# 3dlg-hcvc/tricolo

Hardware: AMD Instinct MI355X
Metric: trimodal training samples/sec (32^3 voxel + 6-view) (higher is better)
Workload: dtype f16 (f16 activation storage + f16 MFMA operands, fp32 accumulate; bf16x3 heads/GRU; within 1e-3 of the fp32 reference)

## Files before the change

tricolo_amd/csrc/conv_pw.hip:

```cpp
#include "common.h"
#include "../../include/tricolo_hip.h"
#include "conv_vox.h"

struct PwArgs {
    const void* in;
    const void* w;
    void* out;
    float* stats;
    int M, K, N, Kpad;
    int GH, GW;
    int transposed;
};

template <int N>
static __device__ __forceinline__ float pw_row_ror(float v) {
    return __builtin_bit_cast(float, __builtin_amdgcn_update_dpp(0, __builtin_bit_cast(int, v), 0x120 + N, 0xf, 0xf, false));
}

template <typename AT, int BN>
__global__ __launch_bounds__(256) void conv_pw_kernel(const PwArgs p) {
    typedef Mma<typename OpOf<AT>::E> MM;
    typedef typename MM::v8 v8;
    constexpr int TN = BN / 16, TM = 2;
    extern __shared__ __attribute__((aligned(16))) char smem[];
    const int t = threadIdx.x, lane = t & 63, wave = t >> 6, fr = lane & 15, fq = lane >> 4;
    const int NT = p.N / BN;
    const int mtile = blockIdx.x / NT, ntile = blockIdx.x - mtile * NT;
    const int K = p.K, kchunks = K >> 3;

    {
        const AT* w = (const AT*)p.w + (size_t)ntile * BN * p.Kpad;
        for (int e = t; e < BN * kchunks; e += 256) {
            const int n = e / kchunks, c = e - n * kchunks;
            const uint4 v = *(const uint4*)(w + (size_t)n * p.Kpad + c * 8);
            *(uint4*)(smem + ((size_t)n * kchunks + (c ^ (n & 7))) * 16) = v;
        }
    }
    const AT* src[TM];
    bool ok[TM];
    size_t opix[TM];
#pragma unroll
    for (int a = 0; a < TM; ++a) {
        const int m = mtile * 128 + wave * 32 + a * 16 + fr;
        ok[a] = m < p.M;
        const int mm = ok[a] ? m : 0;
        const int x = mm % p.GW, q = mm / p.GW, y = q % p.GH, n = q / p.GH;
        const size_t big = (((size_t)n * 2 * p.GH + 2 * y) * 2 * p.GW + 2 * x);
        if (!p.transposed) { src[a] = (const AT*)p.in + big * K; opix[a] = (size_t)mm * p.N; }
        else { src[a] = (const AT*)p.in + (size_t)mm * K; opix[a] = big * p.N; }
    }
    __syncthreads();

    f32x4 acc[TM][TN];
#pragma unroll
    for (int a = 0; a < TM; ++a)
#pragma unroll
        for (int b = 0; b < TN; ++b) acc[a][b] = (f32x4){0.f, 0.f, 0.f, 0.f};
    for (int k0 = 0; k0 < K; k0 += 128) {
        uint4 af[4][TM];
#pragma unroll
        for (int s = 0; s < 4; ++s)
#pragma unroll
            for (int a = 0; a < TM; ++a) {
                af[s][a] = make_uint4(0u, 0u, 0u, 0u);
                if (ok[a] && k0 + s * 32 < K) af[s][a] = *(const uint4*)(src[a] + k0 + s * 32 + fq * 8);
            }
#pragma unroll
        for (int s = 0; s < 4; ++s) {
            if (k0 + s * 32 >= K) break;
            const int c = ((k0 + s * 32) >> 3) + fq;
#pragma unroll
            for (int b = 0; b < TN; ++b) {
                const uint4 bf = *(const uint4*)(smem + ((size_t)(b * 16 + fr) * kchunks + (c ^ (fr & 7))) * 16);
#pragma unroll
                for (int a = 0; a < TM; ++a) acc[a][b] = MM::mma(__builtin_bit_cast(v8, bf), __builtin_bit_cast(v8, af[s][a]), acc[a][b]);
            }
        }
    }

    AT* const out = (AT*)p.out + ntile * BN;
    if (p.transposed) {
        const size_t dx = p.N, dy = (size_t)2 * p.GW * p.N;
        const float4 z = make_float4(0.f, 0.f, 0.f, 0.f);
#pragma unroll
        for (int a = 0; a < TM; ++a) {
            if (!ok[a]) continue;
#pragma unroll
            for (int b = 0; b < TN; ++b) {
                AT* o = out + opix[a] + b * 16 + fq * 4;
                const f32x4 v = acc[a][b];
                Act<AT>::st4(o, make_float4(v[0], v[1], v[2], v[3]));
                Act<AT>::st4(o + dx, z);
                Act<AT>::st4(o + dy, z);
                Act<AT>::st4(o + dy + dx, z);
            }
        }
        return;
    }
    f32x4 cs[TN], cq[TN];
#pragma unroll
    for (int b = 0; b < TN; ++b) { cs[b] = (f32x4){0.f, 0.f, 0.f, 0.f}; cq[b] = cs[b]; }
#pragma unroll
    for (int a = 0; a < TM; ++a) {
        if (!ok[a]) continue;
#pragma unroll
        for (int b = 0; b < TN; ++b) {
            f32x4 v = acc[a][b];
            Act<AT>::st4(out + opix[a] + b * 16 + fq * 4, make_float4(v[0], v[1], v[2], v[3]));
            v[0] = Act<AT>::rnd(v[0]); v[1] = Act<AT>::rnd(v[1]); v[2] = Act<AT>::rnd(v[2]); v[3] = Act<AT>::rnd(v[3]);
            cs[b] += v;
            cq[b] += v * v;
        }
    }
    if (!p.stats) return;
    __syncthreads();
    float* const red = (float*)smem;
#pragma unroll
    for (int b = 0; b < TN; ++b)
#pragma unroll
        for (int r = 0; r < 4; ++r) {
            float s_ = cs[b][r], q_ = cq[b][r];
            s_ += pw_row_ror<8>(s_); q_ += pw_row_ror<8>(q_);
            s_ += pw_row_ror<4>(s_); q_ += pw_row_ror<4>(q_);
            s_ += pw_row_ror<2>(s_); q_ += pw_row_ror<2>(q_);
            s_ += pw_row_ror<1>(s_); q_ += pw_row_ror<1>(q_);
            if (fr == 0) {
                const int col = b * 16 + fq * 4 + r;
                red[(wave * BN + col) * 2 + 0] = s_;
                red[(wave * BN + col) * 2 + 1] = q_;
            }
        }
    __syncthreads();
    if (t < BN) {
        float s_ = 0.f, q_ = 0.f;
#pragma unroll
        for (int w2 = 0; w2 < 4; ++w2) { s_ += red[(w2 * BN + t) * 2]; q_ += red[(w2 * BN + t) * 2 + 1]; }
        p.stats[((size_t)mtile * 2 + 0) * p.N + ntile * BN + t] = s_;
        p.stats[((size_t)mtile * 2 + 1) * p.N + ntile * BN + t] = q_;
    }
}

bool tri_internal_pw_geometry(const TriConvDesc& d, TriPwGeom* g) {
    if (tri_env_is("TRICOLO_NO_PW_CONV", '1') || d.KD != 1 || d.KH != 1 || d.KW != 1 || d.stride != 2 || d.pad_d || d.pad_h || d.pad_w || d.ID != 1 || d.OD != 1) return false;
    if (d.Cin % 64 || d.Cin > 512 || d.Cout % 64) return false;
    int transposed;
    if (d.IH == 2 * d.OH && d.IW == 2 * d.OW) transposed = 0;
    else if (d.OH == 2 * d.IH && d.OW == 2 * d.IW) transposed = 1;
    else return false;
    const int GH = transposed ? d.IH : d.OH, GW = transposed ? d.IW : d.OW;
    const long M = (long)d.B * GH * GW;
    if (M * 4 * (d.Cin > d.Cout ? d.Cin : d.Cout) * 2 >= ((long)1 << 31)) return false;
    const int mtiles = (int)((M + 127) / 128);
    const int bn = (d.Cout % 128 == 0 && (long)128 * d.Cin * 2 <= 65536 && (long)mtiles * (d.Cout / 128) >= 256) ? 128 : 64;
    g->bn = bn; g->mtiles = mtiles; g->GH = GH; g->GW = GW; g->transposed = transposed;
    return true;
}

template <typename AT>
static int pw_launch_t(const TriPwGeom& g, const PwArgs& a, hipStream_t stream) {
    const size_t smem = (size_t)g.bn * a.K * 2 > (size_t)4 * g.bn * 2 * 4 ? (size_t)g.bn * a.K * 2 : (size_t)4 * g.bn * 2 * 4;
    const int grid = g.mtiles * (a.N / g.bn);
    if (g.bn == 128) {
        static bool set = false;
        if (!set) { hipFuncSetAttribute((const void*)conv_pw_kernel<AT, 128>, hipFuncAttributeMaxDynamicSharedMemorySize, 65536); set = true; }
        conv_pw_kernel<AT, 128><<<grid, 256, smem, stream>>>(a);
    } else {
        static bool set = false;
        if (!set) { hipFuncSetAttribute((const void*)conv_pw_kernel<AT, 64>, hipFuncAttributeMaxDynamicSharedMemorySize, 65536); set = true; }
        conv_pw_kernel<AT, 64><<<grid, 256, smem, stream>>>(a);
    }
    return tri_check_launch("tri_conv(pw)");
}

int tri_internal_pw_launch(const TriPwGeom& g, int B, const void* in, const void* w, int K, int N, int Kpad, void* out, float* stats, int transposed,
                           int act_fmt, hipStream_t stream) {
    PwArgs a{};
    a.in = in; a.w = w; a.out = out; a.stats = transposed ? nullptr : stats;
    a.M = B * g.GH * g.GW; a.K = K; a.N = N; a.Kpad = Kpad; a.GH = g.GH; a.GW = g.GW; a.transposed = transposed;
    return act_fmt == TRI_FMT_F16 ? pw_launch_t<f16_t>(g, a, stream) : pw_launch_t<bf16_t>(g, a, stream);
}
```

Before: 13370.

## Prefetch A fragments, coalesce weight staging and transposed stores, add BN=32 tiles

The pointwise stride-2 conv kernel gains a DG variant for the transposed (upsampling) path. It issues the first A-fragment loads before weight staging and double-buffers the next K-chunk's loads during the MFMA loop. Weight staging is rearranged into batched 8-chunk loads, and output is staged through per-wave LDS so each lane writes full 16-byte rows plus the zero fill, giving coalesced scatter. A BN=32 tile is also picked when the grid would otherwise be small, to raise parallelism, at the cost of more register pressure and extra LDS traffic.

```diff
diff --git a/tricolo_amd/csrc/conv_pw.hip b/tricolo_amd/csrc/conv_pw.hip
--- a/tricolo_amd/csrc/conv_pw.hip
+++ b/tricolo_amd/csrc/conv_pw.hip
@@ -17,7 +17,12 @@
     return __builtin_bit_cast(float, __builtin_amdgcn_update_dpp(0, __builtin_bit_cast(int, v), 0x120 + N, 0xf, 0xf, false));
 }
 
-template <typename AT, int BN>
+template <int BN> struct PwStage {
+    static constexpr int PITCH = BN * 2 + 16;
+    static constexpr int WAVE = 32 * PITCH + 32 * 4;
+};
+
+template <typename AT, int BN, bool DG>
 __global__ __launch_bounds__(256) void conv_pw_kernel(const PwArgs p) {
     typedef Mma<typename OpOf<AT>::E> MM;
     typedef typename MM::v8 v8;
@@ -28,17 +33,9 @@
     const int mtile = blockIdx.x / NT, ntile = blockIdx.x - mtile * NT;
     const int K = p.K, kchunks = K >> 3;
 
-    {
-        const AT* w = (const AT*)p.w + (size_t)ntile * BN * p.Kpad;
-        for (int e = t; e < BN * kchunks; e += 256) {
-            const int n = e / kchunks, c = e - n * kchunks;
-            const uint4 v = *(const uint4*)(w + (size_t)n * p.Kpad + c * 8);
-            *(uint4*)(smem + ((size_t)n * kchunks + (c ^ (n & 7))) * 16) = v;
-        }
-    }
     const AT* src[TM];
     bool ok[TM];
-    size_t opix[TM];
+    unsigned opix[TM];
 #pragma unroll
     for (int a = 0; a < TM; ++a) {
         const int m = mtile * 128 + wave * 32 + a * 16 + fr;
@@ -46,8 +43,41 @@
         const int mm = ok[a] ? m : 0;
         const int x = mm % p.GW, q = mm / p.GW, y = q % p.GH, n = q / p.GH;
         const size_t big = (((size_t)n * 2 * p.GH + 2 * y) * 2 * p.GW + 2 * x);
-        if (!p.transposed) { src[a] = (const AT*)p.in + big * K; opix[a] = (size_t)mm * p.N; }
-        else { src[a] = (const AT*)p.in + (size_t)mm * K; opix[a] = big * p.N; }
+        if (!p.transposed) { src[a] = (const AT*)p.in + big * K; opix[a] = (unsigned)((size_t)mm * p.N); }
+        else { src[a] = (const AT*)p.in + (size_t)mm * K; opix[a] = (unsigned)(big * p.N); }
+    }
+#define PW_LOAD_TRIP(af, k0_)                                                                                              \
+    _Pragma("unroll") for (int s = 0; s < 4; ++s)                                                                          \
+        _Pragma("unroll") for (int a = 0; a < TM; ++a) {                                                                   \
+            af[s][a] = make_uint4(0u, 0u, 0u, 0u);                                                                         \
+            if (ok[a] && (k0_) + s * 32 < K) af[s][a] = *(const uint4*)(src[a] + (k0_) + s * 32 + fq * 8);                 \
+        }
+    uint4 cur[4][TM], nxt[4][TM];
+    if (DG) { PW_LOAD_TRIP(cur, 0) }
+    {
+        const AT* w = (const AT*)p.w + (size_t)ntile * BN * p.Kpad;
+        if (!DG) {
+            for (int e = t; e < BN * kchunks; e += 256) {
+                const int n = e / kchunks, c = e - n * kchunks;
+                const uint4 v = *(const uint4*)(w + (size_t)n * p.Kpad + c * 8);
+                *(uint4*)(smem + ((size_t)n * kchunks + (c ^ (n & 7))) * 16) = v;
+            }
+        } else {
+            const int cc = t & 7, ng = kchunks >> 3;
+#pragma unroll
+            for (int i = 0; i < BN / 32; ++i) {
+                const int n = i * 32 + (t >> 3);
+                uint4 v[8];
+#pragma unroll
+                for (int g8 = 0; g8 < 8; ++g8) {
+                    v[g8] = make_uint4(0u, 0u, 0u, 0u);
+                    if (g8 < ng) v[g8] = *(const uint4*)(w + (size_t)n * p.Kpad + (g8 * 8 + cc) * 8);
+                }
+#pragma unroll
+                for (int g8 = 0; g8 < 8; ++g8)
+                    if (g8 < ng) *(uint4*)(smem + ((size_t)n * kchunks + g8 * 8 + (cc ^ (n & 7))) * 16) = v[g8];
+            }
+        }
     }
     __syncthreads();
 
@@ -57,14 +87,9 @@
 #pragma unroll
         for (int b = 0; b < TN; ++b) acc[a][b] = (f32x4){0.f, 0.f, 0.f, 0.f};
     for (int k0 = 0; k0 < K; k0 += 128) {
-        uint4 af[4][TM];
-#pragma unroll
-        for (int s = 0; s < 4; ++s)
-#pragma unroll
-            for (int a = 0; a < TM; ++a) {
-                af[s][a] = make_uint4(0u, 0u, 0u, 0u);
-                if (ok[a] && k0 + s * 32 < K) af[s][a] = *(const uint4*)(src[a] + k0 + s * 32 + fq * 8);
-            }
+        const bool more = DG && k0 + 128 < K;
+        if (!DG) { PW_LOAD_TRIP(cur, k0) }
+        if (more) { PW_LOAD_TRIP(nxt, k0 + 128) }
 #pragma unroll
         for (int s = 0; s < 4; ++s) {
             if (k0 + s * 32 >= K) break;
@@ -73,72 +98,121 @@
             for (int b = 0; b < TN; ++b) {
                 const uint4 bf = *(const uint4*)(smem + ((size_t)(b * 16 + fr) * kchunks + (c ^ (fr & 7))) * 16);
 #pragma unroll
-                for (int a = 0; a < TM; ++a) acc[a][b] = MM::mma(__builtin_bit_cast(v8, bf), __builtin_bit_cast(v8, af[s][a]), acc[a][b]);
-            }
-        }
-    }
-
-    AT* const out = (AT*)p.out + ntile * BN;
-    if (p.transposed) {
-        const size_t dx = p.N, dy = (size_t)2 * p.GW * p.N;
-        const float4 z = make_float4(0.f, 0.f, 0.f, 0.f);
+                for (int a = 0; a < TM; ++a) acc[a][b] = MM::mma(__builtin_bit_cast(v8, bf), __builtin_bit_cast(v8, cur[s][a]), acc[a][b]);
+            }
+        }
+        if (more) {
+#pragma unroll
+            for (int s = 0; s < 4; ++s)
+#pragma unroll
+                for (int a = 0; a < TM; ++a) cur[s][a] = nxt[s][a];
+        }
+    }
+
+    if (!DG) {
+        AT* const out = (AT*)p.out + ntile * BN;
+        if (p.transposed) {
+            const size_t dx = p.N, dy = (size_t)2 * p.GW * p.N;
+            const float4 z = make_float4(0.f, 0.f, 0.f, 0.f);
+#pragma unroll
+            for (int a = 0; a < TM; ++a) {
+                if (!ok[a]) continue;
+#pragma unroll
+                for (int b = 0; b < TN; ++b) {
+                    AT* o = out + opix[a] + b * 16 + fq * 4;
+                    const f32x4 v = acc[a][b];
+                    Act<AT>::st4(o, make_float4(v[0], v[1], v[2], v[3]));
+                    Act<AT>::st4(o + dx, z);
+                    Act<AT>::st4(o + dy, z);
+                    Act<AT>::st4(o + dy + dx, z);
+                }
+            }
+            return;
+        }
+        f32x4 cs[TN], cq[TN];
+#pragma unroll
+        for (int b = 0; b < TN; ++b) { cs[b] = (f32x4){0.f, 0.f, 0.f, 0.f}; cq[b] = cs[b]; }
 #pragma unroll
         for (int a = 0; a < TM; ++a) {
             if (!ok[a]) continue;
 #pragma unroll
             for (int b = 0; b < TN; ++b) {
-                AT* o = out + opix[a] + b * 16 + fq * 4;
-                const f32x4 v = acc[a][b];
-                Act<AT>::st4(o, make_float4(v[0], v[1], v[2], v[3]));
-                Act<AT>::st4(o + dx, z);
-                Act<AT>::st4(o + dy, z);
-                Act<AT>::st4(o + dy + dx, z);
-            }
+                f32x4 v = acc[a][b];
+                Act<AT>::st4(out + opix[a] + b * 16 + fq * 4, make_float4(v[0], v[1], v[2], v[3]));
+                v[0] = Act<AT>::rnd(v[0]); v[1] = Act<AT>::rnd(v[1]); v[2] = Act<AT>::rnd(v[2]); v[3] = Act<AT>::rnd(v[3]);
+                cs[b] += v;
+                cq[b] += v * v;
+            }
+        }
+        if (!p.stats) return;
+        __syncthreads();
+        float* const red = (float*)smem;
+#pragma unroll
+        for (int b = 0; b < TN; ++b)
+#pragma unroll
+            for (int r = 0; r < 4; ++r) {
+                float s_ = cs[b][r], q_ = cq[b][r];
+                s_ += pw_row_ror<8>(s_); q_ += pw_row_ror<8>(q_);
+                s_ += pw_row_ror<4>(s_); q_ += pw_row_ror<4>(q_);
+                s_ += pw_row_ror<2>(s_); q_ += pw_row_ror<2>(q_);
+                s_ += pw_row_ror<1>(s_); q_ += pw_row_ror<1>(q_);
+                if (fr == 0) {
+                    const int col = b * 16 + fq * 4 + r;
+                    red[(wave * BN + col) * 2 + 0] = s_;
+                    red[(wave * BN + col) * 2 + 1] = q_;
+                }
+            }
+        __syncthreads();
+        if (t < BN) {
+            float s_ = 0.f, q_ = 0.f;
+#pragma unroll
+            for (int w2 = 0; w2 < 4; ++w2) { s_ += red[(w2 * BN + t) * 2]; q_ += red[(w2 * BN + t) * 2 + 1]; }
+            p.stats[((size_t)mtile * 2 + 0) * p.N + ntile * BN + t] = s_;
+            p.stats[((size_t)mtile * 2 + 1) * p.N + ntile * BN + t] = q_;
         }
         return;
     }
-    f32x4 cs[TN], cq[TN];
-#pragma unroll
-    for (int b = 0; b < TN; ++b) { cs[b] = (f32x4){0.f, 0.f, 0.f, 0.f}; cq[b] = cs[b]; }
+    __syncthreads();
+    typedef PwStage<BN> ST;
+    char* const stage = smem + wave * ST::WAVE;
+    unsigned* const spix = (unsigned*)(stage + 32 * ST::PITCH);
 #pragma unroll
     for (int a = 0; a < TM; ++a) {
-        if (!ok[a]) continue;
+        if (fq == 0) spix[a * 16 + fr] = ok[a] ? opix[a] : 0xffffffffu;
 #pragma unroll
         for (int b = 0; b < TN; ++b) {
-            f32x4 v = acc[a][b];
-            Act<AT>::st4(out + opix[a] + b * 16 + fq * 4, make_float4(v[0], v[1], v[2], v[3]));
-            v[0] = Act<AT>::rnd(v[0]); v[1] = Act<AT>::rnd(v[1]); v[2] = Act<AT>::rnd(v[2]); v[3] = Act<AT>::rnd(v[3]);
-            cs[b] += v;
-            cq[b] += v * v;
-        }
-    }
-    if (!p.stats) return;
-    __syncthreads();
-    float* const red = (float*)smem;
-#pragma unroll
-    for (int b = 0; b < TN; ++b)
-#pragma unroll
-        for (int r = 0; r < 4; ++r) {
-            float s_ = cs[b][r], q_ = cq[b][r];
-            s_ += pw_row_ror<8>(s_); q_ += pw_row_ror<8>(q_);
-            s_ += pw_row_ror<4>(s_); q_ += pw_row_ror<4>(q_);
-            s_ += pw_row_ror<2>(s_); q_ += pw_row_ror<2>(q_);
-            s_ += pw_row_ror<1>(s_); q_ += pw_row_ror<1>(q_);
-            if (fr == 0) {
-                const int col = b * 16 + fq * 4 + r;
-                red[(wave * BN + col) * 2 + 0] = s_;
-                red[(wave * BN + col) * 2 + 1] = q_;
-            }
-        }
-    __syncthreads();
-    if (t < BN) {
-        float s_ = 0.f, q_ = 0.f;
-#pragma unroll
-        for (int w2 = 0; w2 < 4; ++w2) { s_ += red[(w2 * BN + t) * 2]; q_ += red[(w2 * BN + t) * 2 + 1]; }
-        p.stats[((size_t)mtile * 2 + 0) * p.N + ntile * BN + t] = s_;
-        p.stats[((size_t)mtile * 2 + 1) * p.N + ntile * BN + t] = q_;
-    }
-}
+            const f32x4 v = acc[a][b];
+            Act<AT>::st4((AT*)(stage + (a * 16 + fr) * ST::PITCH) + b * 16 + fq * 4, make_float4(v[0], v[1], v[2], v[3]));
+        }
+    }
+    __builtin_amdgcn_fence(__ATOMIC_ACQ_REL, "workgroup");
+    __builtin_amdgcn_wave_barrier();
+    {
+        constexpr int LPR = BN / 8, RPI = 64 / LPR, NIT = 32 / RPI;
+        AT* const out = (AT*)p.out + ntile * BN + (lane % LPR) * 8;
+        const size_t dx = p.N, dy = (size_t)2 * p.GW * p.N;
+        const uint4 z = make_uint4(0u, 0u, 0u, 0u);
+        unsigned px[NIT];
+        uint4 v[NIT];
+#pragma unroll
+        for (int it = 0; it < NIT; ++it) {
+            const int r = it * RPI + lane / LPR;
+            px[it] = spix[r];
+            v[it] = *(const uint4*)(stage + r * ST::PITCH + (lane % LPR) * 16);
+        }
+#pragma unroll
+        for (int it = 0; it < NIT; ++it) {
+            if (px[it] != 0xffffffffu) {
+                AT* o = out + px[it];
+                *(uint4*)o = v[it];
+                *(uint4*)(o + dx) = z;
+                *(uint4*)(o + dy) = z;
+                *(uint4*)(o + dy + dx) = z;
+            }
+        }
+    }
+}
+#undef PW_LOAD_TRIP
 
 bool tri_internal_pw_geometry(const TriConvDesc& d, TriPwGeom* g) {
     if (tri_env_is("TRICOLO_NO_PW_CONV", '1') || d.KD != 1 || d.KH != 1 || d.KW != 1 || d.stride != 2 || d.pad_d || d.pad_h || d.pad_w || d.ID != 1 || d.OD != 1) return false;
@@ -156,20 +230,23 @@
     return true;
 }
 
+template <typename AT, int BN, bool DG>
+static int pw_launch_bn(const TriPwGeom& g, const PwArgs& a, hipStream_t stream) {
+    size_t smem = (size_t)BN * a.K * 2;
+    if (smem < (size_t)4 * BN * 2 * 4) smem = (size_t)4 * BN * 2 * 4;
+    if (DG && smem < (size_t)4 * PwStage<BN>::WAVE) smem = (size_t)4 * PwStage<BN>::WAVE;
+    static bool set = false;
+    if (!set) { hipFuncSetAttribute((const void*)conv_pw_kernel<AT, BN, DG>, hipFuncAttributeMaxDynamicSharedMemorySize, 65536); set = true; }
+    conv_pw_kernel<AT, BN, DG><<<g.mtiles * (a.N / BN), 256, smem, stream>>>(a);
+    return tri_check_launch("tri_conv(pw)");
+}
+
 template <typename AT>
 static int pw_launch_t(const TriPwGeom& g, const PwArgs& a, hipStream_t stream) {
-    const size_t smem = (size_t)g.bn * a.K * 2 > (size_t)4 * g.bn * 2 * 4 ? (size_t)g.bn * a.K * 2 : (size_t)4 * g.bn * 2 * 4;
-    const int grid = g.mtiles * (a.N / g.bn);
-    if (g.bn == 128) {
-        static bool set = false;
-        if (!set) { hipFuncSetAttribute((const void*)conv_pw_kernel<AT, 128>, hipFuncAttributeMaxDynamicSharedMemorySize, 65536); set = true; }
-        conv_pw_kernel<AT, 128><<<grid, 256, smem, stream>>>(a);
-    } else {
-        static bool set = false;
-        if (!set) { hipFuncSetAttribute((const void*)conv_pw_kernel<AT, 64>, hipFuncAttributeMaxDynamicSharedMemorySize, 65536); set = true; }
-        conv_pw_kernel<AT, 64><<<grid, 256, smem, stream>>>(a);
-    }
-    return tri_check_launch("tri_conv(pw)");
+    if (g.bn == 128) return pw_launch_bn<AT, 128, false>(g, a, stream);
+    const bool cut = (long)g.mtiles * (a.N / 32) <= 512;
+    if (a.transposed) return cut ? pw_launch_bn<AT, 32, true>(g, a, stream) : pw_launch_bn<AT, 64, true>(g, a, stream);
+    return cut ? pw_launch_bn<AT, 32, false>(g, a, stream) : pw_launch_bn<AT, 64, false>(g, a, stream);
 }
 
 int tri_internal_pw_launch(const TriPwGeom& g, int B, const void* in, const void* w, int K, int N, int Kpad, void* out, float* stats, int transposed,
```

Result: no change. 13310 (median of 3 runs) (-0.4%).
